# matinraayai/ir2rgb

Hardware: AMD Instinct MI355X
Metric: generator+discriminator frames/sec at 512x1024 (higher is better)
Workload: dtype bf16; 1 GPU; vid2vid training window 512x1024: 2-scale generator (composite ngf128 @256x512 + composite-local ngf64 @512x1024, tG=3) + FlowNet2 reference flow + image D (num_D=2) + 2 temporal D, 3 backward passes + Adam; batch 1 frame per GPU; parallelism=dp1 (frame-parallel sequences, RCCL gradient all-reduce)

## Files before the change

ir2rgb_amd/csrc/wgrad_mfma.hip:

```cpp
#include <utility>

#include "common.h"

typedef __attribute__((ext_vector_type(8))) short s16x8;

struct WgradGeom {
    int N, Hq, Wq;
    int Hv, Wv;
    int Ca, Cb;
    int stride_y, stride_x, pad_mode;
    int nty, ntx, dy0, dx0;
    int ksplit, ksteps;
    int tpb;
    FastDiv div_hw, div_w;
    unsigned u_bytes, v_bytes;
};

template <int DT>
__device__ __forceinline__ f32x4 mfma_s16(s16x8 a, s16x8 b, f32x4 c) {
    typedef typename Half<DT>::frag frag;
    return Half<DT>::mfma(__builtin_bit_cast(frag, a), __builtin_bit_cast(frag, b), c);
}

__device__ __forceinline__ s16x4 lds_tr(const unsigned char *p) {
    return __builtin_amdgcn_ds_read_tr16_b64_v4i16((__attribute__((address_space(3))) s16x4 *)p);
}

template <int DT>
__global__ void __launch_bounds__(512, 2)
conv_wgrad_kernel(const uint16_t *__restrict__ U, const uint16_t *__restrict__ V, float *__restrict__ D,
                  const WgradGeom g) {
    constexpr int STAGE = 2 * 64 * 256;
    __shared__ __attribute__((aligned(1024))) unsigned char smem[2 * STAGE];

    const int tid0 = threadIdx.x, lane = tid0 & 63;
    const int wave8 = __builtin_amdgcn_readfirstlane(tid0 >> 6);
    const bool loader = wave8 >= 4;
    const int wave = wave8 & 3;
    const int tid = tid0 & 255;
    const int nta = (g.Ca + 127) >> 7, ntb = (g.Cb + 127) >> 7;
    int bid;
    {
        const int nwg = gridDim.x, b = blockIdx.x, xcd = b & 7, q = nwg >> 3, r = nwg & 7;
        bid = (xcd < r ? xcd * (q + 1) : r * (q + 1) + (xcd - r) * q) + (b >> 3);
    }
    const int ntaps = g.nty * g.ntx, ntg = (ntaps + g.tpb - 1) / g.tpb;
    const int tb = bid % ntb; bid /= ntb;
    const int ta = bid % nta; bid /= nta;
    const int tapg = bid % ntg;
    const int split = bid / ntg;
    const int a0 = ta * 128, b0 = tb * 128;
    const int per = (g.ksteps + g.ksplit - 1) / g.ksplit;
    const int kbeg = split * per, kend = min(g.ksteps, kbeg + per);
    if (kbeg >= kend) return;

    const int slot = tid & 15, r0 = tid >> 4;
    const int f = (r0 & 3) | (((r0 >> 3) & 1) << 2);
    const int chunk = ((((slot >> 1) ^ f) << 1) | (slot & 1));
    const int vtap = g.tpb == 2 ? tapg * 2 + (chunk >> 3) : tapg;
    const int vch = g.tpb == 2 ? (chunk & 7) * 8 : b0 + chunk * 8;
    const int ty = vtap / g.ntx, tx = vtap - ty * g.ntx;
    const int dy = g.dy0 + ty, dx = g.dx0 + tx;
    const bool a_ok = a0 + chunk * 8 < g.Ca, b_ok = vch < g.Cb && vtap < ntaps;
    const rsrc_t ru = make_rsrc(U, g.u_bytes), rv = make_rsrc(V, g.v_bytes);
    const unsigned ubase = a_ok ? (unsigned)(a0 + chunk * 8) * 2u : IR2RGB_OOB;
    const unsigned vbase = b_ok ? (unsigned)vch * 2u : IR2RGB_OOB;
    const unsigned Q = (unsigned)g.N * g.Hq * g.Wq, HWq = (unsigned)g.Hq * g.Wq;
    const unsigned ca2 = (unsigned)g.Ca * 2u, cb2 = (unsigned)g.Cb * 2u;
    unsigned char *const wave_dst = smem + wave * 1024;
    const bool wide = g.Wq >= 16;

    auto issue_row = [&](unsigned q, unsigned n, unsigned qy, unsigned qx, unsigned char *dst) {
        const bool v = q < Q;
        lds_dma16(ru, v ? ubase + q * ca2 : IR2RGB_OOB, 0, dst);
        int iy = (int)qy * g.stride_y + dy, ix = (int)qx * g.stride_x + dx;
        const bool inb = ((unsigned)iy < (unsigned)g.Hv) & ((unsigned)ix < (unsigned)g.Wv);
        iy = g.pad_mode ? reflect(iy, g.Hv) : iy;
        ix = g.pad_mode ? reflect(ix, g.Wv) : ix;
        const unsigned vp = (n * (unsigned)g.Hv + (unsigned)iy) * (unsigned)g.Wv + (unsigned)ix;
        lds_dma16(rv, (v && (g.pad_mode || inb)) ? vbase + vp * cb2 : IR2RGB_OOB, 0, dst + 16384);
    };
    auto issue = [&](int ks, int buf) {
        unsigned char *dst = wave_dst + buf * STAGE;
        unsigned q = (unsigned)ks * 64u + r0;
        unsigned qq = q < Q ? q : 0u;
        unsigned n = fdiv(qq, g.div_hw), rem = qq - n * HWq;
        unsigned qy = fdiv(rem, g.div_w), qx = rem - qy * g.Wq;
        if (wide) {
#pragma unroll
            for (int i = 0; i < 4; ++i) {
                issue_row(q, n, qy, qx, dst + 4096 * i);
                q += 16;
                qx += 16;
                const bool wr_ = qx >= (unsigned)g.Wq;
                qx = wr_ ? qx - g.Wq : qx;
                qy += wr_ ? 1u : 0u;
                const bool wy_ = qy >= (unsigned)g.Hq;
                qy = wy_ ? 0u : qy;
                n += wy_ ? 1u : 0u;
            }
        } else {
#pragma unroll
            for (int i = 0; i < 4; ++i) {
                issue_row(q, n, qy, qx, dst + 4096 * i);
                q += 16;
                qq = q < Q ? q : 0u;
                n = fdiv(qq, g.div_hw); rem = qq - n * HWq;
                qy = fdiv(rem, g.div_w); qx = rem - qy * g.Wq;
            }
        }
    };

    const int wr = wave >> 1, wc = wave & 1;
    const int grp = lane >> 4, l15 = lane & 15;
    const int qd = l15 >> 2, pp = l15 & 3;
    const int fr = qd | ((grp & 1) << 2);
    const int lane_off = (8 * grp + qd) * 256 + (pp >> 1) * 16 + (pp & 1) * 8;
    int aoff[4], boff[4];
#pragma unroll
    for (int m = 0; m < 4; ++m) {
        aoff[m] = lane_off + ((((wr * 64 + m * 16) >> 4) ^ fr) << 5);
        boff[m] = lane_off + ((((wc * 64 + m * 16) >> 4) ^ fr) << 5) + 16384;
    }
    auto frag = [&](const unsigned char *p, int kk) -> s16x8 {
        const s16x4 lo = lds_tr(p + (kk * 32) * 256);
        const s16x4 hi = lds_tr(p + (kk * 32 + 4) * 256);
        return (s16x8){lo[0], lo[1], lo[2], lo[3], hi[0], hi[1], hi[2], hi[3]};
    };

    f32x4 acc[4][4];
#pragma unroll
    for (int mi = 0; mi < 4; ++mi)
#pragma unroll
        for (int ni = 0; ni < 4; ++ni) acc[mi][ni] = (f32x4){0.f, 0.f, 0.f, 0.f};

    if (loader) {
        issue(kbeg, 0);
        int lb = 0;
        for (int ks = kbeg; ks < kend; ++ks) {
            asm volatile("s_waitcnt vmcnt(0)" ::: "memory");
            __builtin_amdgcn_s_barrier();
            if (ks + 1 < kend) issue(ks + 1, lb ^ 1);
            lb ^= 1;
        }
        return;
    }
    int buf = 0;
    for (int ks = kbeg; ks < kend; ++ks) {
        __builtin_amdgcn_s_barrier();
        const unsigned char *tile = smem + buf * STAGE;
        const unsigned char *pa[4], *pb[4];
#pragma unroll
        for (int m = 0; m < 4; ++m) { pa[m] = tile + aoff[m]; pb[m] = tile + boff[m]; }
#pragma unroll
        for (int kk = 0; kk < 2; ++kk) {
            s16x8 a[4], b[4];
#pragma unroll
            for (int mi = 0; mi < 4; ++mi) a[mi] = frag(pa[mi], kk);
#pragma unroll
            for (int ni = 0; ni < 4; ++ni) b[ni] = frag(pb[ni], kk);
#pragma unroll
            for (int mi = 0; mi < 4; ++mi)
#pragma unroll
                for (int ni = 0; ni < 4; ++ni) acc[mi][ni] = mfma_s16<DT>(a[mi], b[ni], acc[mi][ni]);
        }
        buf ^= 1;
    }

    const int tap = g.tpb == 2 ? tapg * 2 + wc : tapg;
    if (tap >= ntaps) return;
    float *Dt = D + ((long)split * ntaps + tap) * g.Ca * g.Cb;
#pragma unroll
    for (int mi = 0; mi < 4; ++mi)
#pragma unroll
        for (int ni = 0; ni < 4; ++ni) {
            const int b = g.tpb == 2 ? ni * 16 + l15 : b0 + wc * 64 + ni * 16 + l15;
#pragma unroll
            for (int r = 0; r < 4; ++r) {
                const int a = a0 + wr * 64 + mi * 16 + grp * 4 + r;
                if (a < g.Ca && b < g.Cb) {
                    Dt[(long)a * g.Cb + b] = acc[mi][ni][r];
                }
            }
        }
}

struct Wgrad9Geom {
    int N, H, W, Ca, Cb, pad_mode;
    int ksteps, ksplit, segs;
    unsigned u_bytes, v_bytes;
};

#define W9_STAGE 36864
#define W9_NST 4

template <int IMM>
__device__ __forceinline__ s16x4 tr_read(unsigned lds_addr) {
    s16x4 v;
    asm volatile("ds_read_b64_tr_b16 %0, %1 offset:%2" : "=v"(v) : "v"(lds_addr), "n"(IMM) : "memory");
    return v;
}

template <int DT>
__global__ void __launch_bounds__(512, 1)
conv_wgrad3x3_kernel(const uint16_t *__restrict__ U, const uint16_t *__restrict__ V, float *__restrict__ D,
                     const Wgrad9Geom g) {
    __shared__ __attribute__((aligned(1024))) unsigned char smem[W9_NST * W9_STAGE];
    const int tid = threadIdx.x, lane = tid & 63;
    const int wave8 = __builtin_amdgcn_readfirstlane(tid >> 6);
    const bool loader = wave8 >= 4;
    const int wave = wave8 & 3;
    const int ntb = g.Cb >> 6, nta = g.Ca >> 6;
    int bid = blockIdx.x;
    const int tb = bid % ntb; bid /= ntb;
    const int ta = bid % nta;
    const int split = bid / nta;
    const int a0 = ta * 64, b0 = tb * 64;
    const int per = (g.ksteps + g.ksplit - 1) / g.ksplit;
    const int kbeg = split * per, kend = min(g.ksteps, kbeg + per);

    const rsrc_t ru = make_rsrc(U, g.u_bytes), rv = make_rsrc(V, g.v_bytes);
    const int rin = lane >> 3, sl = lane & 7;
    auto fsw = [](int r) { return ((r >> 1) & 1) | (((r >> 3) & 1) << 1); };
    unsigned u_off[2];
    int v_L0[7], v_fixU[7], v_fixD[7], v_fixL[7], v_fixR[7], v_edge[7];
    bool v_dead[7];
    const int cb2i = g.Cb * 2;
#pragma unroll
    for (int j = 0; j < 2; ++j) {
        const int r = (wave + 4 * j) * 8 + rin;
        const int chunk = (((sl >> 1) ^ fsw(r)) << 1) | (sl & 1);
        u_off[j] = (unsigned)r * (unsigned)g.Ca * 2u + (unsigned)(a0 + chunk * 8) * 2u;
    }
#pragma unroll
    for (int j = 0; j < 7; ++j) {
        const int id = wave + 4 * (j + 2);
        const int R = (id - 8) * 8 + rin;
        const bool real = id < 33 && R < 198;
        const int pr = R / 66, pxl = R - pr * 66;
        const int chunk = (((sl >> 1) ^ fsw(R)) << 1) | (sl & 1);
        const int dy = pr - 1, dx = pxl - 1;
        v_dead[j] = !real;
        v_L0[j] = (dy * g.W + dx) * cb2i + (b0 + chunk * 8) * 2;
        v_fixU[j] = dy == -1 ? 2 * g.W * cb2i : 0;
        v_fixD[j] = dy == 1 ? -2 * g.W * cb2i : 0;
        v_fixL[j] = dx == -1 ? 2 * cb2i : 0;
        v_fixR[j] = dx == 64 ? -2 * cb2i : 0;
        v_edge[j] = (dy == -1 ? 1 : 0) | (dy == 1 ? 2 : 0) | (dx == -1 ? 4 : 0) | (dx == 64 ? 8 : 0);
    }
    const unsigned ca2 = (unsigned)g.Ca * 2u;
    const bool refl = g.pad_mode != 0;
    int is_row = kbeg / g.segs, is_seg = kbeg - is_row * g.segs, is_y = is_row % g.H, is_ks = kbeg;
    auto issue = [&](int st) {
        unsigned char *dst = smem + st * W9_STAGE + wave * 1024;
        const bool live = is_ks < kend;
        const int x0 = is_seg * 64;
        const unsigned pix = (unsigned)is_row * (unsigned)g.W + (unsigned)x0;
        const unsigned ubase = pix * ca2;
        const int vbase = (int)(pix * (unsigned)cb2i);
        const bool top = is_y == 0, bot = is_y == g.H - 1, first = is_seg == 0, last = is_seg == g.segs - 1;
        const int edge = (top ? 1 : 0) | (bot ? 2 : 0) | (first ? 4 : 0) | (last ? 8 : 0);
#pragma unroll
        for (int j = 0; j < 2; ++j) lds_dma16(ru, live ? ubase + u_off[j] : IR2RGB_OOB, 0, dst + 4096 * j);
#pragma unroll
        for (int j = 0; j < 7; ++j) {
            const int o = vbase + v_L0[j] + (top ? v_fixU[j] : 0) + (bot ? v_fixD[j] : 0) + (first ? v_fixL[j] : 0) +
                          (last ? v_fixR[j] : 0);
            const bool off = v_dead[j] | !live | (!refl & ((v_edge[j] & edge) != 0));
            lds_dma16(rv, off ? IR2RGB_OOB : (unsigned)o, 0, dst + 4096 * (j + 2));
        }
        ++is_ks;
        if (++is_seg == g.segs) {
            is_seg = 0;
            ++is_row;
            if (++is_y == g.H) is_y = 0;
        }
    };

    const int grp = lane >> 4, l15 = lane & 15;
    const int qd = l15 >> 2, pp = l15 & 3;
    const int sub = (pp >> 1) * 16 + (pp & 1) * 8;
    const int rl = 8 * grp + qd;
    int aoff[4];
#pragma unroll
    for (int mi = 0; mi < 4; ++mi) aoff[mi] = rl * 128 + ((mi ^ fsw(rl)) << 5) + sub;
    int boff[9][2];
#pragma unroll
    for (int t = 0; t < 9; ++t)
#pragma unroll
        for (int h = 0; h < 2; ++h) {
            const int R = (t / 3) * 66 + (t % 3) + rl + 4 * h;
            boff[t][h] = 8192 + R * 128 + ((wave ^ fsw(R)) << 5) + sub;
        }

    f32x4 acc[9][4];
#pragma unroll
    for (int t = 0; t < 9; ++t)
#pragma unroll
        for (int mi = 0; mi < 4; ++mi) acc[t][mi] = (f32x4){0.f, 0.f, 0.f, 0.f};
    const unsigned lds_base = (unsigned)(__SIZE_TYPE__)((__attribute__((address_space(3))) unsigned char *)smem);

    if (kbeg < kend) {
        if (loader) {
            issue(0);
            issue(1);
            issue(2);
            int st = 0;
            for (int ks = kbeg; ks < kend; ++ks) {
                asm volatile("s_waitcnt vmcnt(18)" ::: "memory");
                __builtin_amdgcn_s_barrier();
                issue((st + 3) & 3);
                st = (st + 1) & 3;
            }
            asm volatile("s_waitcnt vmcnt(0)" ::: "memory");
        } else {
            int st = 0;
            for (int ks = kbeg; ks < kend; ++ks) {
                __builtin_amdgcn_s_barrier();
                const unsigned tbase = lds_base + (unsigned)st * W9_STAGE;
                unsigned av[4], bv[9][2];
    #pragma unroll
                for (int mi = 0; mi < 4; ++mi) av[mi] = tbase + (unsigned)aoff[mi];
    #pragma unroll
                for (int t = 0; t < 9; ++t) { bv[t][0] = tbase + (unsigned)boff[t][0]; bv[t][1] = tbase + (unsigned)boff[t][1]; }
                s16x4 alo[2][4], ahi[2][4], blo[4], bhi[4];
#pragma unroll
                for (int mi = 0; mi < 4; ++mi) {
                    alo[0][mi] = tr_read<0>(av[mi]);
                    ahi[0][mi] = tr_read<512>(av[mi]);
                }
#pragma unroll
                for (int q = 0; q < 3; ++q) {
                    blo[q] = tr_read<0>(bv[q][0]);
                    bhi[q] = tr_read<0>(bv[q][1]);
                }
                auto step = [&]<int S>(std::integral_constant<int, S>) {
                    constexpr int KK = S / 9, T = S % 9, cur = S & 3;
                    if constexpr (S == 5) {
#pragma unroll
                        for (int mi = 0; mi < 4; ++mi) {
                            alo[1][mi] = tr_read<4096>(av[mi]);
                            ahi[1][mi] = tr_read<4096 + 512>(av[mi]);
                        }
                    }
                    if constexpr (S + 3 < 18) {
                        constexpr int S3 = S + 3;
                        blo[S3 & 3] = tr_read<(S3 / 9) * 4096>(bv[S3 % 9][0]);
                        bhi[S3 & 3] = tr_read<(S3 / 9) * 4096>(bv[S3 % 9][1]);
                    }
                    constexpr int after = 2 * ((S + 3 < 18 ? 3 : 17 - S)) + ((S >= 5 && S <= 8) ? 8 : 0);
                    if constexpr (T == 0)
                        asm volatile("s_waitcnt lgkmcnt(%10)"
                                     : "+v"(alo[KK][0]), "+v"(ahi[KK][0]), "+v"(alo[KK][1]), "+v"(ahi[KK][1]), "+v"(alo[KK][2]),
                                       "+v"(ahi[KK][2]), "+v"(alo[KK][3]), "+v"(ahi[KK][3]), "+v"(blo[cur]), "+v"(bhi[cur])
                                     : "n"(after)
                                     : "memory");
                    else
                        asm volatile("s_waitcnt lgkmcnt(%2)" : "+v"(blo[cur]), "+v"(bhi[cur]) : "n"(after) : "memory");
                    const s16x8 b = (s16x8){blo[cur][0], blo[cur][1], blo[cur][2], blo[cur][3],
                                            bhi[cur][0], bhi[cur][1], bhi[cur][2], bhi[cur][3]};
#pragma unroll
                    for (int mi = 0; mi < 4; ++mi) {
                        const s16x8 a = (s16x8){alo[KK][mi][0], alo[KK][mi][1], alo[KK][mi][2], alo[KK][mi][3],
                                                ahi[KK][mi][0], ahi[KK][mi][1], ahi[KK][mi][2], ahi[KK][mi][3]};
                        acc[T][mi] = mfma_s16<DT>(a, b, acc[T][mi]);
                    }
                };
                [&]<int... Ss>(std::integer_sequence<int, Ss...>) { (step(std::integral_constant<int, Ss>{}), ...); }
                (std::make_integer_sequence<int, 18>{});
                st = (st + 1) & 3;
            }
        }
    }
    if (loader) return;

    float *Dt = D + (long)split * 9 * g.Ca * g.Cb;
    const int b = b0 + wave * 16 + l15;
#pragma unroll
    for (int mi = 0; mi < 4; ++mi)
#pragma unroll
        for (int r = 0; r < 4; ++r) {
            const int a = a0 + mi * 16 + grp * 4 + r;
            float *o = Dt + ((long)a * g.Cb + b) * 9;
#pragma unroll
            for (int t = 0; t < 9; ++t) o[t] = acc[t][mi][r];
        }
}

struct WgradLineGeom {
    int N, Hq, Wq, Hv, Wv, Ca, Cb;
    int stride_y, pad_mode, dy0, dx0;
    int segs, ksteps, ksplit, per;
    unsigned u_bytes, v_bytes;
};

template <int DT, int NTY, int NTX, int SX = 1>
__global__ void __launch_bounds__(512, 1)
conv_wgrad_line_kernel(const uint16_t *__restrict__ U, const uint16_t *__restrict__ V, float *__restrict__ D,
                       const WgradLineGeom g) {
    constexpr int NT = NTY * NTX;
    constexpr int PW = SX == 2 ? 64 + ((NTX - 1) >> 1) : 64 + NTX - 1;
    constexpr int PR = NTY * (SX == 2 ? 2 : 1) * PW;
    constexpr int NID = 8 + (PR + 7) / 8;
    constexpr int J = (NID + 3) / 4;
    constexpr int STAGE = NID * 1024;
    static_assert(2 * STAGE <= 160 * 1024 - 1024, "two stages must fit the LDS");
    __shared__ __attribute__((aligned(1024))) unsigned char smem[2 * STAGE];
    const int tid = threadIdx.x, lane = tid & 63;
    const int wave8 = __builtin_amdgcn_readfirstlane(tid >> 6);
    const bool loader = wave8 >= 4;
    const int wave = wave8 & 3;
    const int ntb = g.Cb >> 6, nta = g.Ca >> 6;
    int bid = blockIdx.x;
    const int tb = bid % ntb; bid /= ntb;
    const int ta = bid % nta;
    const int split = bid / nta;
    const int a0 = ta * 64, b0 = tb * 64;
    const int kbeg = split * g.per, kend = min(g.ksteps, kbeg + g.per);
    auto fsw = [](int r) { return ((r >> 1) & 1) | (((r >> 3) & 1) << 1); };

    if (loader) {
        const rsrc_t ru = make_rsrc(U, g.u_bytes), rv = make_rsrc(V, g.v_bytes);
        const int rin = lane >> 3, sl = lane & 7;
        const unsigned ca2 = (unsigned)g.Ca * 2u, cb2 = (unsigned)g.Cb * 2u;
        int is_row = kbeg / g.segs, is_seg = kbeg - is_row * g.segs, is_n = is_row / g.Hq, is_y = is_row - is_n * g.Hq;
        auto issue = [&](int buf) {
            unsigned char *dst = smem + buf * STAGE + wave * 1024;
            const int x0 = is_seg * 64;
#pragma unroll
            for (int j = 0; j < J; ++j) {
                const int id = wave + 4 * j;
                if (id >= NID) break;
                unsigned off = IR2RGB_OOB;
                if (id < 8) {
                    const int r = id * 8 + rin;
                    const int chunk = (((sl >> 1) ^ fsw(r)) << 1) | (sl & 1);
                    if (x0 + r < g.Wq)
                        off = ((unsigned)is_row * (unsigned)g.Wq + (unsigned)(x0 + r)) * ca2 + (unsigned)(a0 + chunk * 8) * 2u;
                    lds_dma16(ru, off, 0, dst + 4096 * j);
                } else {
                    const int R = (id - 8) * 8 + rin;
                    const int run = R / PW, pxl = R - run * PW;
                    const int pr = SX == 2 ? run >> 1 : run;
                    const int chunk = (((sl >> 1) ^ fsw(R)) << 1) | (sl & 1);
                    int iy = is_y * g.stride_y + g.dy0 + pr;
                    int ix = SX == 2 ? 2 * x0 + g.dx0 + 2 * pxl + (run & 1) : x0 + pxl + g.dx0;
                    const bool inb = ((unsigned)iy < (unsigned)g.Hv) & ((unsigned)ix < (unsigned)g.Wv);
                    iy = g.pad_mode ? reflect(iy, g.Hv) : iy;
                    ix = g.pad_mode ? reflect(ix, g.Wv) : ix;
                    ix = min(max(ix, 0), g.Wv - 1);
                    iy = min(max(iy, 0), g.Hv - 1);
                    if (R < PR && (g.pad_mode || inb))
                        off = (((unsigned)is_n * (unsigned)g.Hv + (unsigned)iy) * (unsigned)g.Wv + (unsigned)ix) * cb2 +
                              (unsigned)(b0 + chunk * 8) * 2u;
                    lds_dma16(rv, off, 0, dst + 4096 * j);
                }
            }
            if (++is_seg == g.segs) {
                is_seg = 0;
                ++is_row;
                if (++is_y == g.Hq) { is_y = 0; ++is_n; }
            }
        };
        issue(0);
        int lb = 0;
        for (int ks = kbeg; ks < kend; ++ks) {
            asm volatile("s_waitcnt vmcnt(0)" ::: "memory");
            __builtin_amdgcn_s_barrier();
            if (ks + 1 < kend) issue(lb ^ 1);
            lb ^= 1;
        }
        return;
    }

    const int grp = lane >> 4, l15 = lane & 15;
    const int qd = l15 >> 2, pp = l15 & 3;
    const int sub = (pp >> 1) * 16 + (pp & 1) * 8;
    const int rl = 8 * grp + qd;
    int aoff[4];
#pragma unroll
    for (int mi = 0; mi < 4; ++mi) aoff[mi] = rl * 128 + ((mi ^ fsw(rl)) << 5) + sub;
    int boff[NT][2];
#pragma unroll
    for (int t = 0; t < NT; ++t)
#pragma unroll
        for (int h = 0; h < 2; ++h) {
            const int ty = t / NTX, tx = t % NTX;
            const int R = (SX == 2 ? (ty * 2 + (tx & 1)) * PW + (tx >> 1) : ty * PW + tx) + rl + 4 * h;
            boff[t][h] = 8192 + R * 128 + ((wave ^ fsw(R)) << 5) + sub;
        }
    f32x4 acc[NT][4];
#pragma unroll
    for (int t = 0; t < NT; ++t)
#pragma unroll
        for (int mi = 0; mi < 4; ++mi) acc[t][mi] = (f32x4){0.f, 0.f, 0.f, 0.f};
    int buf = 0;
    for (int ks = kbeg; ks < kend; ++ks) {
        __builtin_amdgcn_s_barrier();
        const unsigned char *tile = smem + buf * STAGE;
#pragma unroll
        for (int kk = 0; kk < 2; ++kk) {
            s16x8 a[4];
#pragma unroll
            for (int mi = 0; mi < 4; ++mi) {
                const s16x4 lo = lds_tr(tile + aoff[mi] + kk * 4096), hi = lds_tr(tile + aoff[mi] + kk * 4096 + 512);
                a[mi] = (s16x8){lo[0], lo[1], lo[2], lo[3], hi[0], hi[1], hi[2], hi[3]};
            }
#pragma unroll
            for (int t = 0; t < NT; ++t) {
                const s16x4 lo = lds_tr(tile + boff[t][0] + kk * 4096), hi = lds_tr(tile + boff[t][1] + kk * 4096);
                const s16x8 b = (s16x8){lo[0], lo[1], lo[2], lo[3], hi[0], hi[1], hi[2], hi[3]};
#pragma unroll
                for (int mi = 0; mi < 4; ++mi) acc[t][mi] = mfma_s16<DT>(a[mi], b, acc[t][mi]);
            }
        }
        asm volatile("s_waitcnt lgkmcnt(0)" ::: "memory");
        buf ^= 1;
    }
    const int b = b0 + wave * 16 + l15;
#pragma unroll
    for (int t = 0; t < NT; ++t) {
        float *Dt = D + ((long)split * NT + t) * g.Ca * g.Cb;
#pragma unroll
        for (int mi = 0; mi < 4; ++mi)
#pragma unroll
            for (int r = 0; r < 4; ++r) Dt[(long)(a0 + mi * 16 + grp * 4 + r) * g.Cb + b] = acc[t][mi][r];
    }
}

template <int DT, int NTY, int SY>
__global__ void __launch_bounds__(512, 1)
conv_wgrad_col_kernel(const uint16_t *__restrict__ U, const uint16_t *__restrict__ V, float *__restrict__ D,
                      const WgradLineGeom g) {
    constexpr int RC = NTY + SY;
    constexpr int PATCH0 = 16384;
    constexpr int LDS = PATCH0 + 2 * RC * 8192;
    constexpr int JMAX = (8 + NTY * 8 + 3) / 4;
    static_assert(LDS <= 160 * 1024 - 1024, "ring must fit the LDS");
    __shared__ __attribute__((aligned(1024))) unsigned char smem[LDS];
    const int tid = threadIdx.x, lane = tid & 63;
    const int wave8 = __builtin_amdgcn_readfirstlane(tid >> 6);
    const bool loader = wave8 >= 4;
    const int wave = wave8 & 3;
    const int ntb = g.Cb >> 6, nta = g.Ca >> 6;
    int bid = blockIdx.x;
    const int tb = bid % ntb; bid /= ntb;
    const int ta = bid % nta;
    const int split = bid / nta;
    const int a0 = ta * 64, b0 = tb * 64;
    const int kbeg = split * g.per, kend = min(g.ksteps, kbeg + g.per);
    auto fsw = [](int r) { return ((r >> 1) & 1) | (((r >> 3) & 1) << 1); };

    if (loader) {
        const rsrc_t ru = make_rsrc(U, g.u_bytes), rv = make_rsrc(V, g.v_bytes);
        const int rin = lane >> 3, sl = lane & 7;
        const unsigned ca2 = (unsigned)g.Ca * 2u, cb2 = (unsigned)g.Cb * 2u;
        int col = kbeg / g.Hq, y = kbeg - col * g.Hq, n = col / g.segs, seg = col - n * g.segs, ub = 0;
        bool first = true;
        auto issue = [&]() {
            const bool prime = first || y == 0;
            const int x0 = seg * 64, half = col & 1;
            const int total = 8 + (prime ? NTY : SY) * 8;
#pragma unroll
            for (int j = 0; j < JMAX; ++j) {
                const int id = wave + 4 * j;
                if (id >= total) break;
                unsigned off = IR2RGB_OOB;
                if (id < 8) {
                    const int r = id * 8 + rin;
                    const int chunk = (((sl >> 1) ^ fsw(r)) << 1) | (sl & 1);
                    if (x0 + r < g.Wq)
                        off = (((unsigned)n * (unsigned)g.Hq + (unsigned)y) * (unsigned)g.Wq + (unsigned)(x0 + r)) * ca2 +
                              (unsigned)(a0 + chunk * 8) * 2u;
                    lds_dma16(ru, off, 0, smem + ub * 8192 + id * 1024);
                } else {
                    const int q = id - 8;
                    const int jt = (prime ? 0 : NTY - SY) + (q >> 3);
                    const int r = (q & 7) * 8 + rin;
                    const int chunk = (((sl >> 1) ^ fsw(r)) << 1) | (sl & 1);
                    const int v = y * SY + jt;
                    int iy = v + g.dy0;
                    const int ix = x0 + r;
                    const bool inb = ((unsigned)iy < (unsigned)g.Hv) & (ix < g.Wv);
                    iy = g.pad_mode ? reflect(iy, g.Hv) : iy;
                    iy = min(max(iy, 0), g.Hv - 1);
                    if (ix < g.Wv && (g.pad_mode || inb))
                        off = (((unsigned)n * (unsigned)g.Hv + (unsigned)iy) * (unsigned)g.Wv + (unsigned)ix) * cb2 +
                              (unsigned)(b0 + chunk * 8) * 2u;
                    const int slot = half * RC + v % RC;
                    lds_dma16(rv, off, 0, smem + PATCH0 + slot * 8192 + (q & 7) * 1024);
                }
            }
            first = false;
            ub ^= 1;
            if (++y == g.Hq) {
                y = 0;
                ++col;
                if (++seg == g.segs) { seg = 0; ++n; }
            }
        };
        issue();
        for (int ks = kbeg; ks < kend; ++ks) {
            asm volatile("s_waitcnt vmcnt(0)" ::: "memory");
            __builtin_amdgcn_s_barrier();
            if (ks + 1 < kend) issue();
        }
        return;
    }

    const int grp = lane >> 4, l15 = lane & 15;
    const int qd = l15 >> 2, pp = l15 & 3;
    const int sub = (pp >> 1) * 16 + (pp & 1) * 8;
    const int rl = 8 * grp + qd;
    int aoff[4], boffl[2];
#pragma unroll
    for (int mi = 0; mi < 4; ++mi) aoff[mi] = rl * 128 + ((mi ^ fsw(rl)) << 5) + sub;
#pragma unroll
    for (int h = 0; h < 2; ++h) boffl[h] = PATCH0 + (rl + 4 * h) * 128 + ((wave ^ fsw(rl + 4 * h)) << 5) + sub;
    f32x4 acc[NTY][4];
#pragma unroll
    for (int t = 0; t < NTY; ++t)
#pragma unroll
        for (int mi = 0; mi < 4; ++mi) acc[t][mi] = (f32x4){0.f, 0.f, 0.f, 0.f};
    int col = kbeg / g.Hq, y = kbeg - col * g.Hq, ub = 0;
    for (int ks = kbeg; ks < kend; ++ks) {
        __builtin_amdgcn_s_barrier();
        const unsigned char *ut = smem + ub * 8192;
        const int base = (col & 1) * RC, v0 = (y * SY) % RC;
#pragma unroll
        for (int kk = 0; kk < 2; ++kk) {
            s16x8 a[4];
#pragma unroll
            for (int mi = 0; mi < 4; ++mi) {
                const s16x4 lo = lds_tr(ut + aoff[mi] + kk * 4096), hi = lds_tr(ut + aoff[mi] + kk * 4096 + 512);
                a[mi] = (s16x8){lo[0], lo[1], lo[2], lo[3], hi[0], hi[1], hi[2], hi[3]};
            }
#pragma unroll
            for (int t = 0; t < NTY; ++t) {
                int slot = v0 + t;
                slot = slot >= RC ? slot - RC : slot;
                const unsigned char *pt = smem + (base + slot) * 8192 + kk * 4096;
                const s16x4 lo = lds_tr(pt + boffl[0]), hi = lds_tr(pt + boffl[1]);
                const s16x8 b = (s16x8){lo[0], lo[1], lo[2], lo[3], hi[0], hi[1], hi[2], hi[3]};
#pragma unroll
                for (int mi = 0; mi < 4; ++mi) acc[t][mi] = mfma_s16<DT>(a[mi], b, acc[t][mi]);
            }
        }
        asm volatile("s_waitcnt lgkmcnt(0)" ::: "memory");
        ub ^= 1;
        if (++y == g.Hq) { y = 0; ++col; }
    }
    const int b = b0 + wave * 16 + l15;
#pragma unroll
    for (int t = 0; t < NTY; ++t) {
        float *Dt = D + ((long)split * NTY + t) * g.Ca * g.Cb;
#pragma unroll
        for (int mi = 0; mi < 4; ++mi)
#pragma unroll
            for (int r = 0; r < 4; ++r) Dt[(long)(a0 + mi * 16 + grp * 4 + r) * g.Cb + b] = acc[t][mi][r];
    }
}

__global__ void __launch_bounds__(256)
wgrad_sum_kernel(const float4 *__restrict__ D, float4 *__restrict__ out, long n4, int nsplit) {
    for (long i = blockIdx.x * (long)blockDim.x + threadIdx.x; i < n4; i += (long)gridDim.x * blockDim.x) {
        float4 s = D[i];
#pragma unroll 4
        for (int k = 1; k < nsplit; ++k) {
            const float4 v = D[k * n4 + i];
            s.x += v.x; s.y += v.y; s.z += v.z; s.w += v.w;
        }
        out[i] = s;
    }
}

static bool plan9(const ir2rgb_conv_desc *d, Wgrad9Geom *g) {
    if (d->transposed || d->kh != 3 || d->kw != 3 || d->stride_h != 1 || d->stride_w != 1 || d->pad_h != 1 || d->pad_w != 1)
        return false;
    if (d->Hout != d->Hin || d->Wout != d->Win || (d->Win % 64) || (d->Cin % 64) || (d->Cout % 64) || d->Hin < 2) return false;
    const long Q = (long)d->N * d->Hin * d->Win;
    if (Q * d->Cout * 2 >= (1L << 31) || Q * d->Cin * 2 >= (1L << 31)) return false;
    *g = Wgrad9Geom{};
    g->N = d->N; g->H = d->Hin; g->W = d->Win; g->Ca = d->Cout; g->Cb = d->Cin; g->pad_mode = d->pad_mode;
    g->segs = d->Win / 64;
    g->ksteps = (int)(Q / 64);
    g->u_bytes = (unsigned)(Q * d->Cout * 2); g->v_bytes = (unsigned)(Q * d->Cin * 2);
    const long tiles = (long)(d->Cout / 64) * (d->Cin / 64);
    long ks = (256 + tiles - 1) / tiles;
    if (ks > g->ksteps / 8) ks = g->ksteps / 8;
    if (ks < 1) ks = 1;
    if (ks > 256) ks = 256;
    g->ksplit = (int)ks;
    return true;
}

__global__ void __launch_bounds__(256)
wgrad_finish_kernel(const float *__restrict__ D, float *__restrict__ out, int Ca, int Cb, int ntaps, int nsplit,
                    long total, int acc) {
    const long slab = (long)ntaps * Ca * Cb;
    for (long i = blockIdx.x * (long)blockDim.x + threadIdx.x; i < total; i += (long)gridDim.x * blockDim.x) {
        const int tap = (int)(i % ntaps);
        const long ab = i / ntaps;
        const float *p = D + (long)tap * Ca * Cb + ab;
        float s = 0.f;
        for (int k = 0; k < nsplit; ++k) s += p[k * slab];
        out[i] = acc ? out[i] + s : s;
    }
}

#define WF_MAX_TAPS 16
__global__ void __launch_bounds__(256)
wgrad_finish_tiled_kernel(const float *__restrict__ D, float *__restrict__ out, long AB, int ntaps, int nsplit, int acc) {
    __shared__ float t[64 * (WF_MAX_TAPS + 1)];
    const int l = threadIdx.x & 63, w = threadIdx.x >> 6;
    const long ab0 = blockIdx.x * 64L, ab = ab0 + l;
    const long slab = (long)ntaps * AB;
    for (int tap = w; tap < ntaps; tap += 4) {
        float s = 0.f;
        if (ab < AB) {
            const float *p = D + (long)tap * AB + ab;
#pragma unroll 8
            for (int k = 0; k < nsplit; ++k) s += p[k * slab];
        }
        t[l * (ntaps + 1) + tap] = s;
    }
    __syncthreads();
    const long left = AB - ab0;
    const int n = (int)(left < 64 ? left : 64) * ntaps;
    for (int j = threadIdx.x; j < n; j += 256) {
        const float v = t[(j / ntaps) * (ntaps + 1) + j % ntaps];
        out[ab0 * ntaps + j] = acc ? out[ab0 * ntaps + j] + v : v;
    }
}

__global__ void __launch_bounds__(256)
wgrad_finish_wide_kernel(const float *__restrict__ D, float *__restrict__ out, long AB, int ntaps, int nsplit, int acc) {
    __shared__ float part[4][64];
    const int l = threadIdx.x & 63, w = threadIdx.x >> 6, tap = blockIdx.y;
    const long ab = blockIdx.x * 64L + l;
    const long slab = (long)ntaps * AB;
    float s = 0.f;
    if (ab < AB) {
        const float *p = D + (long)tap * AB + ab;
#pragma unroll 8
        for (int k = w; k < nsplit; k += 4) s += p[k * slab];
    }
    part[w][l] = s;
    __syncthreads();
    if (w == 0 && ab < AB) {
        const float v = ((part[0][l] + part[1][l]) + part[2][l]) + part[3][l];
        const long o = ab * ntaps + tap;
        out[o] = acc ? out[o] + v : v;
    }
}

static void launch_wgrad_finish(const float *D, float *out, int Ca, int Cb, int ntaps, int nsplit, hipStream_t s, int acc = 0) {
    const long AB = (long)Ca * Cb, elems = AB * ntaps;
    if (nsplit > 64 && (AB + 63) / 64 <= 0x7fffffffL && ntaps <= 65535)
        wgrad_finish_wide_kernel<<<dim3((unsigned)((AB + 63) / 64), (unsigned)ntaps), 256, 0, s>>>(D, out, AB, ntaps, nsplit, acc);
    else if (ntaps <= WF_MAX_TAPS && (AB + 63) / 64 <= 0x7fffffffL)
        wgrad_finish_tiled_kernel<<<(unsigned)((AB + 63) / 64), 256, 0, s>>>(D, out, AB, ntaps, nsplit, acc);
    else
        wgrad_finish_kernel<<<stream_grid(elems, 256), 256, 0, s>>>(D, out, Ca, Cb, ntaps, nsplit, elems, acc);
}

static int plan(const ir2rgb_conv_desc *d, WgradGeom *g) {
    if (!d || d->N < 1 || d->Cin < 8 || d->Cout < 8 || (d->Cin % 8) || (d->Cout % 8) || d->kh < 1 || d->kw < 1 ||
        d->stride_h < 1 || d->stride_w < 1 || d->pad_h < 0 || d->pad_w < 0)
        return IR2RGB_EINVAL;
    if (d->dtype != IR2RGB_BF16 && d->dtype != IR2RGB_F16) return IR2RGB_ENOSUP;
    if (d->transposed && d->pad_mode != 0) return IR2RGB_ENOSUP;
    *g = WgradGeom{};
    g->N = d->N;
    if (!d->transposed) {
        g->Hq = d->Hout; g->Wq = d->Wout; g->Hv = d->Hin; g->Wv = d->Win; g->Ca = d->Cout; g->Cb = d->Cin;
    } else {
        g->Hq = d->Hin; g->Wq = d->Win; g->Hv = d->Hout; g->Wv = d->Wout; g->Ca = d->Cin; g->Cb = d->Cout;
    }
    g->stride_y = d->stride_h; g->stride_x = d->stride_w; g->pad_mode = d->pad_mode;
    g->nty = d->kh; g->ntx = d->kw; g->dy0 = -d->pad_h; g->dx0 = -d->pad_w;
    long Q = (long)g->N * g->Hq * g->Wq;
    if (Q >= (1L << 31) || (long)g->N * g->Hv * g->Wv >= (1L << 31)) return IR2RGB_EINVAL;
    g->ksteps = (int)((Q + 63) / 64);
    g->tpb = (g->Cb <= 64 && d->kh * d->kw > 1) ? 2 : 1;
    const long tiles = (long)((d->kh * d->kw + g->tpb - 1) / g->tpb) * ((g->Ca + 127) / 128) * ((g->Cb + 127) / 128);
    const double elems = (double)d->kh * d->kw * g->Ca * g->Cb;
    int best = 1;
    double best_cost = 1e30;
    for (int ks = 1; ks <= 64; ++ks) {
        if (ks > 1 && g->ksteps / ks < 4) break;
        const double rounds = (double)((tiles * ks + 511) / 512);
        const double cost = rounds * ((g->ksteps + ks - 1) / ks + 3) * 1.2 + ks * elems * 8.0 / 4e6;
        if (cost < best_cost) { best_cost = cost; best = ks; }
    }
    g->ksplit = best;
    g->div_hw = make_fastdiv((unsigned)(g->Hq * g->Wq)); g->div_w = make_fastdiv((unsigned)g->Wq);
    {
        const long ub = Q * g->Ca * 2, vb = (long)g->N * g->Hv * g->Wv * g->Cb * 2;
        if (ub >= (1L << 31) || vb >= (1L << 31)) return IR2RGB_EINVAL;
        g->u_bytes = (unsigned)ub; g->v_bytes = (unsigned)vb;
    }
    return IR2RGB_OK;
}

static bool plan_line(const ir2rgb_conv_desc *d, WgradLineGeom *g) {
    if ((d->Cin % 64) || (d->Cout % 64)) return false;
    const long tl = (long)(d->Cout / 64) * (d->Cin / 64);
    const bool k3s2 = d->kh == 3 && d->kw == 3 && d->stride_h == 2 && d->stride_w == 2 && d->pad_mode == 0 && (tl <= 2 || tl >= 128);
    const bool k7x1 = d->kh == 7 && d->kw == 1, k1x7 = d->kh == 1 && d->kw == 7, k4x1 = d->kh == 4 && d->kw == 1;
    if (!k3s2 && (d->transposed || d->stride_w != 1)) return false;
    if (!(k7x1 || k1x7 || k4x1 || k3s2)) return false;
    if (k7x1 && d->pad_w != 0) return false;
    if (k4x1 && d->pad_w != 0) return false;
    if (d->pad_mode != 0 && d->pad_mode != 1) return false;
    if (d->pad_mode == 1 && (d->pad_h >= d->Hin || d->pad_w >= d->Win)) return false;
    *g = WgradLineGeom{};
    g->N = d->N;
    if (!d->transposed) {
        g->Hq = d->Hout; g->Wq = d->Wout; g->Hv = d->Hin; g->Wv = d->Win; g->Ca = d->Cout; g->Cb = d->Cin;
    } else {
        g->Hq = d->Hin; g->Wq = d->Win; g->Hv = d->Hout; g->Wv = d->Wout; g->Ca = d->Cin; g->Cb = d->Cout;
    }
    const long Q = (long)d->N * g->Hq * g->Wq, Pv = (long)d->N * g->Hv * g->Wv;
    if (Q * g->Ca * 2 >= (1L << 31) || Pv * g->Cb * 2 >= (1L << 31)) return false;
    g->stride_y = d->stride_h; g->pad_mode = d->pad_mode; g->dy0 = -d->pad_h; g->dx0 = -d->pad_w;
    g->segs = (g->Wq + 63) / 64;
    const long ksteps = (long)d->N * g->Hq * g->segs;
    if (ksteps >= (1L << 30)) return false;
    g->ksteps = (int)ksteps;
    const long tiles = (long)(g->Ca / 64) * (g->Cb / 64);
    long ks = (256 + tiles - 1) / tiles;
    if (ks > ksteps / 8) ks = ksteps / 8;
    if (ks < 1) ks = 1;
    if (ks > 256) ks = 256;
    g->per = (int)((ksteps + ks - 1) / ks);
    g->ksplit = (int)((ksteps + g->per - 1) / g->per);
    g->u_bytes = (unsigned)(Q * g->Ca * 2); g->v_bytes = (unsigned)(Pv * g->Cb * 2);
    return true;
}

template <int DT>
static void launch_line(const ir2rgb_conv_desc *d, const WgradLineGeom &g, const uint16_t *U, const uint16_t *V, float *D, hipStream_t s) {
    const unsigned grid = (unsigned)((long)g.ksplit * (g.Ca / 64) * (g.Cb / 64));
    if (d->kh == 3 && d->kw == 3) conv_wgrad_line_kernel<DT, 3, 3, 2><<<grid, 512, 0, s>>>(U, V, D, g);
    else if (d->kh == 7 && d->stride_h == 1) conv_wgrad_col_kernel<DT, 7, 1><<<grid, 512, 0, s>>>(U, V, D, g);
    else if (d->kh == 4 && d->stride_h == 2) conv_wgrad_col_kernel<DT, 4, 2><<<grid, 512, 0, s>>>(U, V, D, g);
    else if (d->kh == 7) conv_wgrad_line_kernel<DT, 7, 1><<<grid, 512, 0, s>>>(U, V, D, g);
    else if (d->kw == 7) conv_wgrad_line_kernel<DT, 1, 7><<<grid, 512, 0, s>>>(U, V, D, g);
    else conv_wgrad_line_kernel<DT, 4, 1><<<grid, 512, 0, s>>>(U, V, D, g);
}

extern "C" long ir2rgb_conv2d_wgrad_workspace_elems(const ir2rgb_conv_desc *d) {
    WgradGeom g;
    int rc = plan(d, &g);
    if (rc) return rc;
    Wgrad9Geom g9;
    if (plan9(d, &g9)) return g9.ksplit > 1 ? (long)g9.ksplit * 9 * g9.Ca * g9.Cb : 4;
    WgradLineGeom gl;
    if (plan_line(d, &gl)) return (long)gl.ksplit * d->kh * d->kw * gl.Ca * gl.Cb;
    return (long)g.ksplit * d->kh * d->kw * g.Ca * g.Cb;
}

static int wgrad_impl(const ir2rgb_conv_desc *d, const void *x, const void *gy, float *dw, float *workspace, void *stream,
                      int acc);

extern "C" int ir2rgb_conv2d_wgrad(const ir2rgb_conv_desc *d, const void *x, const void *gy, float *dw,
                                   float *workspace, void *stream) {
    return wgrad_impl(d, x, gy, dw, workspace, stream, 0);
}

extern "C" int ir2rgb_conv2d_wgrad_acc(const ir2rgb_conv_desc *d, const void *x, const void *gy, float *dw,
                                       float *workspace, void *stream) {
    return wgrad_impl(d, x, gy, dw, workspace, stream, 1);
}

extern "C" long ir2rgb_conv2d_wgrad_acc_workspace_elems(const ir2rgb_conv_desc *d) {
    WgradGeom g;
    int rc = plan(d, &g);
    if (rc) return rc;
    WgradLineGeom gl;
    if (plan_line(d, &gl)) return (long)gl.ksplit * d->kh * d->kw * gl.Ca * gl.Cb;
    return (long)g.ksplit * d->kh * d->kw * g.Ca * g.Cb;
}

static int wgrad_impl(const ir2rgb_conv_desc *d, const void *x, const void *gy, float *dw, float *workspace, void *stream,
                      int acc) {
    WgradGeom g;
    int rc = plan(d, &g);
    if (rc) return rc;
    if ((((uintptr_t)x | (uintptr_t)gy) & 15) || !dw || !workspace) return IR2RGB_EALIGN;
    hipStream_t s = as_stream(stream);
    const int ntaps = d->kh * d->kw;
    const long elems = (long)ntaps * g.Ca * g.Cb;
    Wgrad9Geom g9;
    if (!acc && plan9(d, &g9)) {
        if (((uintptr_t)dw | (uintptr_t)workspace) & 15) return IR2RGB_EALIGN;
        float *dst = g9.ksplit > 1 ? workspace : dw;
        const unsigned grid9 = (unsigned)((long)g9.ksplit * (g9.Ca / 64) * (g9.Cb / 64));
        if (d->dtype == IR2RGB_BF16) conv_wgrad3x3_kernel<IR2RGB_BF16><<<grid9, 512, 0, s>>>((const uint16_t *)gy, (const uint16_t *)x, dst, g9);
        else conv_wgrad3x3_kernel<IR2RGB_F16><<<grid9, 512, 0, s>>>((const uint16_t *)gy, (const uint16_t *)x, dst, g9);
        if (g9.ksplit > 1)
            wgrad_sum_kernel<<<stream_grid(elems / 4, 256), 256, 0, s>>>((const float4 *)workspace, (float4 *)dw, elems / 4, g9.ksplit);
        return ir2rgb_launch_status();
    }
    const uint16_t *U = (const uint16_t *)(d->transposed ? x : gy), *V = (const uint16_t *)(d->transposed ? gy : x);
    WgradLineGeom gl;
    if (plan_line(d, &gl)) {
        if (d->dtype == IR2RGB_BF16) launch_line<IR2RGB_BF16>(d, gl, U, V, workspace, s);
        else launch_line<IR2RGB_F16>(d, gl, U, V, workspace, s);
        launch_wgrad_finish(workspace, dw, gl.Ca, gl.Cb, ntaps, gl.ksplit, s, acc);
        return ir2rgb_launch_status();
    }
    const unsigned grid = (unsigned)((long)g.ksplit * ((ntaps + g.tpb - 1) / g.tpb) * ((g.Ca + 127) / 128) * ((g.Cb + 127) / 128));
    if (d->dtype == IR2RGB_BF16) conv_wgrad_kernel<IR2RGB_BF16><<<grid, 512, 0, s>>>(U, V, workspace, g);
    else conv_wgrad_kernel<IR2RGB_F16><<<grid, 512, 0, s>>>(U, V, workspace, g);
    launch_wgrad_finish(workspace, dw, g.Ca, g.Cb, ntaps, g.ksplit, s, acc);
    return ir2rgb_launch_status();
}
```

Baseline: 39.73 frames/s.

## Add dedicated stride-2 wgrad kernel with 3-stage LDS ring and tap grouping

Moves stride-2 3x3 and 4x4 weight-gradient convolutions out of the generic line kernel into a new dedicated kernel. The new kernel uses a deeper (up to 3-stage) LDS ring with vmcnt-based waits, precomputes per-lane loader address state, remaps blocks across XCDs, and splits 4x4 taps into two groups. It also writes the result directly when no k-split is needed, which skips the reduction pass. The goal is to hide global-load latency and widen coverage, including transposed 3x3 stride-2 and 4x4 downsampling convs. The cost is more code and a more complex split heuristic.

```diff
diff --git a/ir2rgb_amd/csrc/wgrad_mfma.hip b/ir2rgb_amd/csrc/wgrad_mfma.hip
--- a/ir2rgb_amd/csrc/wgrad_mfma.hip
+++ b/ir2rgb_amd/csrc/wgrad_mfma.hip
@@ -1,6 +1,7 @@
 #include <utility>
 
 #include "common.h"
+#include "wgrad_s2.h"
 
 typedef __attribute__((ext_vector_type(8))) short s16x8;
 
@@ -394,13 +395,13 @@
     unsigned u_bytes, v_bytes;
 };
 
-template <int DT, int NTY, int NTX, int SX = 1>
+template <int DT, int NTY, int NTX>
 __global__ void __launch_bounds__(512, 1)
 conv_wgrad_line_kernel(const uint16_t *__restrict__ U, const uint16_t *__restrict__ V, float *__restrict__ D,
                        const WgradLineGeom g) {
     constexpr int NT = NTY * NTX;
-    constexpr int PW = SX == 2 ? 64 + ((NTX - 1) >> 1) : 64 + NTX - 1;
-    constexpr int PR = NTY * (SX == 2 ? 2 : 1) * PW;
+    constexpr int PW = 64 + NTX - 1;
+    constexpr int PR = NTY * PW;
     constexpr int NID = 8 + (PR + 7) / 8;
     constexpr int J = (NID + 3) / 4;
     constexpr int STAGE = NID * 1024;
@@ -440,11 +441,10 @@
                     lds_dma16(ru, off, 0, dst + 4096 * j);
                 } else {
                     const int R = (id - 8) * 8 + rin;
-                    const int run = R / PW, pxl = R - run * PW;
-                    const int pr = SX == 2 ? run >> 1 : run;
+                    const int pr = R / PW, pxl = R - pr * PW;
                     const int chunk = (((sl >> 1) ^ fsw(R)) << 1) | (sl & 1);
                     int iy = is_y * g.stride_y + g.dy0 + pr;
-                    int ix = SX == 2 ? 2 * x0 + g.dx0 + 2 * pxl + (run & 1) : x0 + pxl + g.dx0;
+                    int ix = x0 + pxl + g.dx0;
                     const bool inb = ((unsigned)iy < (unsigned)g.Hv) & ((unsigned)ix < (unsigned)g.Wv);
                     iy = g.pad_mode ? reflect(iy, g.Hv) : iy;
                     ix = g.pad_mode ? reflect(ix, g.Wv) : ix;
@@ -486,7 +486,7 @@
 #pragma unroll
         for (int h = 0; h < 2; ++h) {
             const int ty = t / NTX, tx = t % NTX;
-            const int R = (SX == 2 ? (ty * 2 + (tx & 1)) * PW + (tx >> 1) : ty * PW + tx) + rl + 4 * h;
+            const int R = ty * PW + tx + rl + 4 * h;
             boff[t][h] = 8192 + R * 128 + ((wave ^ fsw(R)) << 5) + sub;
         }
     f32x4 acc[NT][4];
@@ -661,6 +661,144 @@
     }
 }
 
+template <int DT, int NTY, int NTX>
+__global__ void __launch_bounds__(512, 1)
+conv_wgrad_s2_kernel(const uint16_t *__restrict__ U, const uint16_t *__restrict__ V, float *__restrict__ D,
+                     const WgradS2Geom g) {
+    constexpr int NT = NTY * NTX;
+    constexpr int PR = NTY * 2 * S2_PW;
+    constexpr int NID = 8 + (PR + 7) / 8;
+    constexpr int J = (NID + 3) / 4;
+    constexpr int STAGE = 4 * J * 1024;
+    constexpr int NST = (160 * 1024 - 1024) / STAGE >= 3 ? 3 : 2;
+    static_assert(NST * STAGE <= 160 * 1024 - 1024, "the ring must fit the LDS");
+    static_assert(64 + (NTX - 1) / 2 == S2_PW && (NST - 2) * J < 64, "patch run length / vmcnt range");
+    __shared__ __attribute__((aligned(1024))) unsigned char smem[NST * STAGE];
+    const int tid = threadIdx.x, lane = tid & 63;
+    const int wave8 = __builtin_amdgcn_readfirstlane(tid >> 6);
+    const bool loader = wave8 >= 4;
+    const int wave = wave8 & 3;
+    const int ntb = g.Cb >> 6, nta = g.Ca >> 6;
+    int bid;
+    {
+        const int nwg = gridDim.x, b = blockIdx.x, xcd = b & 7, q = nwg >> 3, r = nwg & 7;
+        bid = (xcd < r ? xcd * (q + 1) : r * (q + 1) + (xcd - r) * q) + (b >> 3);
+    }
+    const int tb = bid % ntb; bid /= ntb;
+    const int ta = bid % nta; bid /= nta;
+    const int grp_t = bid % g.ngroups;
+    const int split = bid / g.ngroups;
+    const int a0 = ta * 64, b0 = tb * 64, ty0 = grp_t * NTY;
+    const int kbeg = split * g.per, kend = min(g.ksteps, kbeg + g.per);
+
+    if (loader) {
+        const rsrc_t ru = make_rsrc(U, g.u_bytes), rv = make_rsrc(V, g.v_bytes);
+        const int rin = lane >> 3, sl = lane & 7;
+        S2Lane lc[J];
+#pragma unroll
+        for (int j = 2; j < J; ++j) lc[j] = s2_lane(NTY, (wave + 4 * j - 8) * 8 + rin, sl, b0);
+        int is_ks = kbeg, is_row = kbeg / g.segs, is_seg = kbeg - is_row * g.segs, is_n = is_row / g.Hq, is_y = is_row - is_n * g.Hq;
+        auto issue = [&](int st) {
+            unsigned char *dst = smem + st * STAGE + wave * 1024;
+            const bool live = is_ks < kend;
+            const int x0 = is_seg * 64;
+#pragma unroll
+            for (int j = 0; j < 2; ++j) {
+                const unsigned off = s2_u_off(g, is_row, x0, (wave + 4 * j) * 8 + rin, sl, a0);
+                lds_dma16(ru, live ? off : S2_OOB, 0, dst + 4096 * j);
+            }
+            const int iy0 = 2 * is_y + g.dy0 + ty0, ix0 = 2 * x0 + g.dx0;
+#pragma unroll
+            for (int j = 2; j < J; ++j) {
+                const unsigned off = s2_v_off(g, lc[j], is_n, iy0, ix0);
+                lds_dma16(rv, live ? off : S2_OOB, 0, dst + 4096 * j);
+            }
+            ++is_ks;
+            if (++is_seg == g.segs) {
+                is_seg = 0;
+                ++is_row;
+                if (++is_y == g.Hq) { is_y = 0; ++is_n; }
+            }
+        };
+#pragma unroll
+        for (int i = 0; i < NST - 1; ++i) issue(i);
+        int st = NST - 1;
+        for (int ks = kbeg; ks < kend; ++ks) {
+            asm volatile("s_waitcnt vmcnt(%0)" ::"n"((NST - 2) * J) : "memory");
+            __builtin_amdgcn_s_barrier();
+            issue(st);
+            st = st + 1 == NST ? 0 : st + 1;
+        }
+        asm volatile("s_waitcnt vmcnt(0)" ::: "memory");
+        return;
+    }
+
+    const int grp = lane >> 4, l15 = lane & 15;
+    const int qd = l15 >> 2, pp = l15 & 3;
+    const int sub = (pp >> 1) * 16 + (pp & 1) * 8;
+    const int rl = 8 * grp + qd;
+    int aoff[4];
+#pragma unroll
+    for (int mi = 0; mi < 4; ++mi) aoff[mi] = rl * 128 + ((mi ^ s2_fsw(rl)) << 5) + sub;
+    int boff[NT][2];
+#pragma unroll
+    for (int t = 0; t < NT; ++t)
+#pragma unroll
+        for (int h = 0; h < 2; ++h) {
+            const int ty = t / NTX, tx = t % NTX;
+            const int R = (ty * 2 + (tx & 1)) * S2_PW + (tx >> 1) + rl + 4 * h;
+            boff[t][h] = 8192 + R * 128 + ((wave ^ s2_fsw(R)) << 5) + sub;
+        }
+    f32x4 acc[NT][4];
+#pragma unroll
+    for (int t = 0; t < NT; ++t)
+#pragma unroll
+        for (int mi = 0; mi < 4; ++mi) acc[t][mi] = (f32x4){0.f, 0.f, 0.f, 0.f};
+    int st = 0;
+    for (int ks = kbeg; ks < kend; ++ks) {
+        __builtin_amdgcn_s_barrier();
+        const unsigned char *tile = smem + st * STAGE;
+#pragma unroll
+        for (int kk = 0; kk < 2; ++kk) {
+            s16x8 a[4];
+#pragma unroll
+            for (int mi = 0; mi < 4; ++mi) {
+                const s16x4 lo = lds_tr(tile + aoff[mi] + kk * 4096), hi = lds_tr(tile + aoff[mi] + kk * 4096 + 512);
+                a[mi] = (s16x8){lo[0], lo[1], lo[2], lo[3], hi[0], hi[1], hi[2], hi[3]};
+            }
+#pragma unroll
+            for (int t = 0; t < NT; ++t) {
+                const s16x4 lo = lds_tr(tile + boff[t][0] + kk * 4096), hi = lds_tr(tile + boff[t][1] + kk * 4096);
+                const s16x8 b = (s16x8){lo[0], lo[1], lo[2], lo[3], hi[0], hi[1], hi[2], hi[3]};
+#pragma unroll
+                for (int mi = 0; mi < 4; ++mi) acc[t][mi] = mfma_s16<DT>(a[mi], b, acc[t][mi]);
+            }
+        }
+        asm volatile("s_waitcnt lgkmcnt(0)" ::: "memory");
+        st = st + 1 == NST ? 0 : st + 1;
+    }
+    const int b = b0 + wave * 16 + l15, ntaps = g.kh * g.kw, tap0 = ty0 * NTX;
+    if (g.direct) {
+#pragma unroll
+        for (int mi = 0; mi < 4; ++mi)
+#pragma unroll
+            for (int r = 0; r < 4; ++r) {
+                float *o = D + ((long)(a0 + mi * 16 + grp * 4 + r) * g.Cb + b) * ntaps + tap0;
+#pragma unroll
+                for (int t = 0; t < NT; ++t) o[t] = acc[t][mi][r];
+            }
+        return;
+    }
+#pragma unroll
+    for (int t = 0; t < NT; ++t) {
+        float *Dt = D + ((long)split * ntaps + tap0 + t) * g.Ca * g.Cb;
+#pragma unroll
+        for (int mi = 0; mi < 4; ++mi)
+#pragma unroll
+            for (int r = 0; r < 4; ++r) Dt[(long)(a0 + mi * 16 + grp * 4 + r) * g.Cb + b] = acc[t][mi][r];
+    }
+}
+
 __global__ void __launch_bounds__(256)
 wgrad_sum_kernel(const float4 *__restrict__ D, float4 *__restrict__ out, long n4, int nsplit) {
     for (long i = blockIdx.x * (long)blockDim.x + threadIdx.x; i < n4; i += (long)gridDim.x * blockDim.x) {
@@ -805,22 +943,16 @@
 
 static bool plan_line(const ir2rgb_conv_desc *d, WgradLineGeom *g) {
     if ((d->Cin % 64) || (d->Cout % 64)) return false;
-    const long tl = (long)(d->Cout / 64) * (d->Cin / 64);
-    const bool k3s2 = d->kh == 3 && d->kw == 3 && d->stride_h == 2 && d->stride_w == 2 && d->pad_mode == 0 && (tl <= 2 || tl >= 128);
     const bool k7x1 = d->kh == 7 && d->kw == 1, k1x7 = d->kh == 1 && d->kw == 7, k4x1 = d->kh == 4 && d->kw == 1;
-    if (!k3s2 && (d->transposed || d->stride_w != 1)) return false;
-    if (!(k7x1 || k1x7 || k4x1 || k3s2)) return false;
+    if (d->transposed || d->stride_w != 1) return false;
+    if (!(k7x1 || k1x7 || k4x1)) return false;
     if (k7x1 && d->pad_w != 0) return false;
     if (k4x1 && d->pad_w != 0) return false;
     if (d->pad_mode != 0 && d->pad_mode != 1) return false;
     if (d->pad_mode == 1 && (d->pad_h >= d->Hin || d->pad_w >= d->Win)) return false;
     *g = WgradLineGeom{};
     g->N = d->N;
-    if (!d->transposed) {
-        g->Hq = d->Hout; g->Wq = d->Wout; g->Hv = d->Hin; g->Wv = d->Win; g->Ca = d->Cout; g->Cb = d->Cin;
-    } else {
-        g->Hq = d->Hin; g->Wq = d->Win; g->Hv = d->Hout; g->Wv = d->Wout; g->Ca = d->Cin; g->Cb = d->Cout;
-    }
+    g->Hq = d->Hout; g->Wq = d->Wout; g->Hv = d->Hin; g->Wv = d->Win; g->Ca = d->Cout; g->Cb = d->Cin;
     const long Q = (long)d->N * g->Hq * g->Wq, Pv = (long)d->N * g->Hv * g->Wv;
     if (Q * g->Ca * 2 >= (1L << 31) || Pv * g->Cb * 2 >= (1L << 31)) return false;
     g->stride_y = d->stride_h; g->pad_mode = d->pad_mode; g->dy0 = -d->pad_h; g->dx0 = -d->pad_w;
@@ -842,12 +974,23 @@
 template <int DT>
 static void launch_line(const ir2rgb_conv_desc *d, const WgradLineGeom &g, const uint16_t *U, const uint16_t *V, float *D, hipStream_t s) {
     const unsigned grid = (unsigned)((long)g.ksplit * (g.Ca / 64) * (g.Cb / 64));
-    if (d->kh == 3 && d->kw == 3) conv_wgrad_line_kernel<DT, 3, 3, 2><<<grid, 512, 0, s>>>(U, V, D, g);
-    else if (d->kh == 7 && d->stride_h == 1) conv_wgrad_col_kernel<DT, 7, 1><<<grid, 512, 0, s>>>(U, V, D, g);
+    if (d->kh == 7 && d->stride_h == 1) conv_wgrad_col_kernel<DT, 7, 1><<<grid, 512, 0, s>>>(U, V, D, g);
     else if (d->kh == 4 && d->stride_h == 2) conv_wgrad_col_kernel<DT, 4, 2><<<grid, 512, 0, s>>>(U, V, D, g);
     else if (d->kh == 7) conv_wgrad_line_kernel<DT, 7, 1><<<grid, 512, 0, s>>>(U, V, D, g);
     else if (d->kw == 7) conv_wgrad_line_kernel<DT, 1, 7><<<grid, 512, 0, s>>>(U, V, D, g);
     else conv_wgrad_line_kernel<DT, 4, 1><<<grid, 512, 0, s>>>(U, V, D, g);
+}
+
+static void launch_s2(const ir2rgb_conv_desc *d, const WgradS2Geom &g, const uint16_t *U, const uint16_t *V, float *D, hipStream_t s) {
+    const unsigned grid = (unsigned)((long)g.ksplit * g.ngroups * (g.Ca / 64) * (g.Cb / 64));
+    const bool bf = d->dtype == IR2RGB_BF16;
+    if (d->kh == 3) {
+        if (bf) conv_wgrad_s2_kernel<IR2RGB_BF16, 3, 3><<<grid, 512, 0, s>>>(U, V, D, g);
+        else conv_wgrad_s2_kernel<IR2RGB_F16, 3, 3><<<grid, 512, 0, s>>>(U, V, D, g);
+    } else {
+        if (bf) conv_wgrad_s2_kernel<IR2RGB_BF16, 2, 4><<<grid, 512, 0, s>>>(U, V, D, g);
+        else conv_wgrad_s2_kernel<IR2RGB_F16, 2, 4><<<grid, 512, 0, s>>>(U, V, D, g);
+    }
 }
 
 extern "C" long ir2rgb_conv2d_wgrad_workspace_elems(const ir2rgb_conv_desc *d) {
@@ -856,6 +999,8 @@
     if (rc) return rc;
     Wgrad9Geom g9;
     if (plan9(d, &g9)) return g9.ksplit > 1 ? (long)g9.ksplit * 9 * g9.Ca * g9.Cb : 4;
+    WgradS2Geom g2;
+    if (plan_s2(d, 0, &g2)) return s2_workspace_elems(g2);
     WgradLineGeom gl;
     if (plan_line(d, &gl)) return (long)gl.ksplit * d->kh * d->kw * gl.Ca * gl.Cb;
     return (long)g.ksplit * d->kh * d->kw * g.Ca * g.Cb;
@@ -878,6 +1023,8 @@
     WgradGeom g;
     int rc = plan(d, &g);
     if (rc) return rc;
+    WgradS2Geom g2;
+    if (plan_s2(d, 1, &g2)) return s2_workspace_elems(g2);
     WgradLineGeom gl;
     if (plan_line(d, &gl)) return (long)gl.ksplit * d->kh * d->kw * gl.Ca * gl.Cb;
     return (long)g.ksplit * d->kh * d->kw * g.Ca * g.Cb;
@@ -904,6 +1051,13 @@
         return ir2rgb_launch_status();
     }
     const uint16_t *U = (const uint16_t *)(d->transposed ? x : gy), *V = (const uint16_t *)(d->transposed ? gy : x);
+    WgradS2Geom g2;
+    if (plan_s2(d, acc, &g2)) {
+        if (g2.direct && (((uintptr_t)dw) & 15)) return IR2RGB_EALIGN;
+        launch_s2(d, g2, U, V, g2.direct ? dw : workspace, s);
+        if (!g2.direct) launch_wgrad_finish(workspace, dw, g2.Ca, g2.Cb, ntaps, g2.ksplit, s, acc);
+        return ir2rgb_launch_status();
+    }
     WgradLineGeom gl;
     if (plan_line(d, &gl)) {
         if (d->dtype == IR2RGB_BF16) launch_line<IR2RGB_BF16>(d, gl, U, V, workspace, s);
diff --git a/ir2rgb_amd/csrc/wgrad_s2.h b/ir2rgb_amd/csrc/wgrad_s2.h
--- /dev/null
+++ b/ir2rgb_amd/csrc/wgrad_s2.h
@@ -0,0 +1,90 @@
+#pragma once
+#include "../../include/ir2rgb_hip.h"
+
+#if defined(__HIPCC__)
+#define S2_HD __host__ __device__ __forceinline__
+#else
+#define S2_HD inline
+#endif
+
+#define S2_OOB 0x80000000u
+#define S2_PW 65
+
+struct WgradS2Geom {
+    int N, Hq, Wq;
+    int Hv, Wv;
+    int Ca, Cb;
+    int kh, kw, dy0, dx0;
+    int ix_last;
+    int ngroups, nty;
+    int segs, ksteps, ksplit, per;
+    int direct;
+    unsigned u_bytes, v_bytes;
+};
+
+static inline bool plan_s2(const ir2rgb_conv_desc *d, int acc, WgradS2Geom *g) {
+    if (!((d->kh == 3 && d->kw == 3) || (d->kh == 4 && d->kw == 4))) return false;
+    if (d->stride_h != 2 || d->stride_w != 2 || d->pad_mode != 0 || d->pad_h < 0 || d->pad_w < 0) return false;
+    if ((d->Cin % 64) || (d->Cout % 64) || d->Cin < 64 || d->Cout < 64 || d->N < 1) return false;
+    *g = WgradS2Geom{};
+    g->N = d->N;
+    if (!d->transposed) {
+        g->Hq = d->Hout; g->Wq = d->Wout; g->Hv = d->Hin; g->Wv = d->Win; g->Ca = d->Cout; g->Cb = d->Cin;
+    } else {
+        g->Hq = d->Hin; g->Wq = d->Win; g->Hv = d->Hout; g->Wv = d->Wout; g->Ca = d->Cin; g->Cb = d->Cout;
+    }
+    if (g->Hq < 1 || g->Wq < 1 || g->Hv < 1 || g->Wv < 1) return false;
+    const long Q = (long)d->N * g->Hq * g->Wq, Pv = (long)d->N * g->Hv * g->Wv;
+    if (Q * g->Ca * 2 >= (1L << 31) || Pv * g->Cb * 2 >= (1L << 31)) return false;
+    if (d->kh == 4 && (d->transposed || g->Wq < 256)) return false;
+    g->kh = d->kh; g->kw = d->kw; g->dy0 = -d->pad_h; g->dx0 = -d->pad_w;
+    g->ix_last = 2 * (g->Wq - 1) + g->dx0 + d->kw - 1;
+    g->ngroups = d->kh == 4 ? 2 : 1;
+    g->nty = d->kh / g->ngroups;
+    g->segs = (g->Wq + 63) / 64;
+    const long ksteps = (long)d->N * g->Hq * g->segs;
+    if (ksteps >= (1L << 30)) return false;
+    g->ksteps = (int)ksteps;
+    const long tiles = (long)(g->Ca / 64) * (g->Cb / 64) * g->ngroups;
+    long ks = (256 + tiles - 1) / tiles;
+    if (ks > ksteps / 8) ks = ksteps / 8;
+    if (ks < 1) ks = 1;
+    if (ks > 256) ks = 256;
+    g->per = (int)((ksteps + ks - 1) / ks);
+    g->ksplit = (int)((ksteps + g->per - 1) / g->per);
+    g->direct = g->ksplit == 1 && !acc;
+    g->u_bytes = (unsigned)(Q * g->Ca * 2); g->v_bytes = (unsigned)(Pv * g->Cb * 2);
+    return true;
+}
+
+static inline long s2_workspace_elems(const WgradS2Geom &g) {
+    return g.direct ? 4 : (long)g.ksplit * g.kh * g.kw * g.Ca * g.Cb;
+}
+
+S2_HD int s2_fsw(int r) { return ((r >> 1) & 1) | (((r >> 3) & 1) << 1); }
+S2_HD int s2_chunk(int r, int sl) { return (((sl >> 1) ^ s2_fsw(r)) << 1) | (sl & 1); }
+
+S2_HD unsigned s2_u_off(const WgradS2Geom &g, int row, int x0, int r, int sl, int a0) {
+    if (x0 + r >= g.Wq) return S2_OOB;
+    return ((unsigned)row * (unsigned)g.Wq + (unsigned)(x0 + r)) * ((unsigned)g.Ca * 2u) + (unsigned)(a0 + s2_chunk(r, sl) * 8) * 2u;
+}
+
+struct S2Lane {
+    int pr, col, ch2;
+    int dead;
+};
+S2_HD S2Lane s2_lane(int nty, int R, int sl, int b0) {
+    S2Lane c;
+    const int run = R / S2_PW, idx = R - run * S2_PW;
+    c.pr = run >> 1;
+    c.col = 2 * idx + (run & 1);
+    c.ch2 = (b0 + s2_chunk(R, sl) * 8) * 2;
+    c.dead = R >= nty * 2 * S2_PW;
+    return c;
+}
+S2_HD unsigned s2_v_off(const WgradS2Geom &g, const S2Lane &c, int n, int iy0, int ix0) {
+    const int iy = iy0 + c.pr, ix = ix0 + c.col;
+    const bool in = ((unsigned)iy < (unsigned)g.Hv) & ((unsigned)ix < (unsigned)g.Wv) & (ix <= g.ix_last) & !c.dead;
+    const unsigned o = (((unsigned)n * (unsigned)g.Hv + (unsigned)iy) * (unsigned)g.Wv + (unsigned)ix) * ((unsigned)g.Cb * 2u) + (unsigned)c.ch2;
+    return in ? o : S2_OOB;
+}
```

After: 39.52 frames/s. About the same (-0.5%).
